# ykojima4020/mae_clip

Measured on NVIDIA B200. Metric: contrastive loss fwd+bwd samples/s, higher is better.
Workload: dtype fp32 (fp16 hi+lo split operands, 3 tcgen05 passes, fp32 accumulate)

## Files before the change

mae_clip_b200/csrc/clip_loss_tc.cu:

```cuda
#include <stdlib.h>
#include <string.h>

#include "clip_loss.cuh"
#include "tc_ptx.cuh"

#include <type_traits>

namespace mc {
namespace tc {

using namespace ptx;


constexpr int kTileN = 128;
constexpr int kRowsCta = 64;
constexpr int kChunkBytes = 64 * 128;
constexpr int kThreads = 384;
constexpr int kEpiThreads = 256;
constexpr int kMaxSplit = 16;
constexpr int kIssuers = 1;

enum Phase { kStats = 0, kRowLoss = 1, kBwd = 2, kStatsZ = 3, kBwdW = 4, kBwdP = 5 };

constexpr int kOffA = 0;
// ... 1206 lines not shown
                                                           float* __restrict__ dT, float* __restrict__ dI,
                                                           const int* __restrict__ gate = nullptr, int gate_want = 0) {
  if (gate != nullptr && *gate != gate_want) return;
  const float scale = (grad_loss ? *grad_loss : 1.f) * inv_2B / *wscale;
  const size_t n4 = (size_t)b * D / 4;
  const size_t plane = (size_t)bpad * D;
  for (size_t i = (size_t)blockIdx.x * blockDim.x + threadIdx.x; i < n4; i += (size_t)gridDim.x * blockDim.x) {
    float4 at = make_float4(0.f, 0.f, 0.f, 0.f), ai = at;
    for (int s = 0; s < nsplit; ++s) {
      const float4 a = reinterpret_cast<const float4*>(part + (size_t)s * 2 * plane)[i];
      const float4 c = reinterpret_cast<const float4*>(part + ((size_t)s * 2 + 1) * plane)[i];
      at.x += a.x; at.y += a.y; at.z += a.z; at.w += a.w;
      ai.x += c.x; ai.y += c.y; ai.z += c.z; ai.w += c.w;
    }
    reinterpret_cast<float4*>(dT)[i] = make_float4(at.x * scale, at.y * scale, at.z * scale, at.w * scale);
    reinterpret_cast<float4*>(dI)[i] = make_float4(ai.x * scale, ai.y * scale, ai.z * scale, ai.w * scale);
  }
}

constexpr int kCgThreads = 256;
constexpr int kCgStageA = 2 * 8192;
constexpr int kCgStages = 6;
constexpr int kCgMaxSplit = 8;
struct ColGradParams {
  int Bp, D;
  int w_rows;
  int row_offset;
  int j_first;
  int n_jblocks;
  int j_end;
  int ksplit, steps_per_split, steps;
  float* part;
  const int* gate;
};
__device__ __forceinline__ uint64_t smem_desc_mn_sw128(uint32_t saddr, uint32_t lbo_bytes) {
  uint64_t d = 0;
  d |= static_cast<uint64_t>((saddr & 0x3FFFFu) >> 4);
  d |= static_cast<uint64_t>(lbo_bytes >> 4) << 16;
  d |= static_cast<uint64_t>(1024 >> 4) << 32;
  d |= static_cast<uint64_t>(1) << 46;
  d |= static_cast<uint64_t>(2) << 61;
  return d;
}
__global__ void __launch_bounds__(kCgThreads, 1)
colgrad_kernel(const __grid_constant__ CUtensorMap map_w, const __grid_constant__ CUtensorMap map_t,
               const ColGradParams p) {
  if (p.gate != nullptr && *p.gate != 1) return;
  extern __shared__ uint8_t smem_raw[];
  const uint32_t raw = smem_u32(smem_raw);
  const uint32_t base = (raw + 1023u) & ~1023u;
  uint8_t* const sbase = smem_raw + (base - raw);
  const int D = p.D;
  const uint32_t b_bytes = (uint32_t)(D / 2) * 128u;
  const uint32_t stage_bytes = kCgStageA + b_bytes;
  const uint32_t bar0 = base + kCgStages * stage_bytes;
  auto bar = [&](int i) -> uint32_t { return bar0 + 8u * i; };
  enum { kFull = 0, kEmpty = kCgStages, kAccFull = 2 * kCgStages, kAccEmpty = 2 * kCgStages + 2, kBars = 2 * kCgStages + 4 };
  uint32_t* const tmem_slot = reinterpret_cast<uint32_t*>(sbase + kCgStages * stage_bytes + 8 * kBars);

  const int warp = __shfl_sync(0xffffffffu, (int)(threadIdx.x >> 5), 0), lane = threadIdx.x & 31;
  const uint32_t rank = cluster_ctarank();
  const bool leader = rank == 0;
  const int pair_id = blockIdx.x >> 1, npairs = gridDim.x >> 1;
  const int njobs = p.n_jblocks * p.ksplit;

  if (threadIdx.x == 0) {
    for (int s = 0; s < kCgStages; ++s) { mbar_init(bar(kFull + s), 1); mbar_init(bar(kEmpty + s), 1); }
    for (int i = 0; i < 2; ++i) { mbar_init(bar(kAccFull + i), 1); mbar_init(bar(kAccEmpty + i), 2 * 128); }
    fence_mbar_init();
    prefetch_tmap(&map_w);
    prefetch_tmap(&map_t);
  }
  if (warp == 1) {
    tmem_alloc_pair(smem_u32(tmem_slot), 512);
    tmem_relinquish_pair();
  }
  tc_fence_before();
  cluster_sync_all();
  tc_fence_after();
  const uint32_t tmem_base = *tmem_slot;

  if (warp == 0) {
    if (elect_one()) {
      uint32_t it = 0;
      for (int job = pair_id; job < njobs; job += npairs) {
        const int jb = job / p.ksplit, ks = job % p.ksplit;
        const int j0 = p.j_first + jb * 256 + (int)rank * 128;
        const int s0 = ks * p.steps_per_split, s1 = min(s0 + p.steps_per_split, p.steps);
        for (int st = s0; st < s1; ++st, ++it) {
          const uint32_t slot = it % kCgStages, par = (it / kCgStages) & 1;
          mbar_wait(bar(kEmpty + slot), par ^ 1);
          const uint32_t fb = bar(kFull + slot), sa = base + slot * stage_bytes;
          if (leader) mbar_arrive_expect_tx(fb, 2u * stage_bytes);
          const int i0 = st * 64;
          tma_load_2d_pair(sa, &map_w, fb, j0, i0);
          tma_load_2d_pair(sa + 8192, &map_w, fb, j0 + 64, i0);
          tma_load_2d_pair(sa + kCgStageA, &map_t, fb, p.row_offset + i0, D + (int)rank * (D / 2));
        }
      }
    }
  } else if (warp == 1) {
    if (leader && elect_one()) {
      const uint32_t idesc = idesc_f16(256, D) | (1u << 15);
      uint32_t it = 0, jj = 0;
      for (int job = pair_id; job < njobs; job += npairs) {
        const int ks = job % p.ksplit;
        const int s0 = ks * p.steps_per_split, s1 = min(s0 + p.steps_per_split, p.steps);
        if (s0 >= s1) continue;
        const uint32_t buf = jj & 1, use = jj >> 1;
        ++jj;
        mbar_wait(bar(kAccEmpty + buf), (use & 1) ^ 1);
        tc_fence_after();
        const uint32_t tacc = tmem_base + buf * (uint32_t)D;
        for (int st = s0; st < s1; ++st, ++it) {
          const uint32_t slot = it % kCgStages, par = (it / kCgStages) & 1;
          mbar_wait(bar(kFull + slot), par);
          tc_fence_after();
          const uint32_t sa = base + slot * stage_bytes;
          const uint64_t bd = smem_desc_sw128(sa + kCgStageA);
#pragma unroll
          for (int k4 = 0; k4 < 4; ++k4)
            mma_f16_pair(tacc, smem_desc_mn_sw128(sa + k4 * 2048, 8192), desc_advance_k(bd, k4), idesc,
                         (st > s0 || k4 > 0) ? 1u : 0u);
          mma_commit_pair(bar(kEmpty + slot), 3);
        }
        mma_commit_pair(bar(kAccFull + buf), 3);
      }
    }
  } else if (warp >= 4) {
// ... 82 lines not shown
                                                                int rows, int D, float inv_2B,
                                                                const float* __restrict__ grad_loss,
                                                                const float* __restrict__ wscale,
                                                                const float* __restrict__ dIz, float* __restrict__ dI,
                                                                const int* __restrict__ gate) {
  if (gate != nullptr && *gate != 1) return;
  const float scale = (grad_loss ? *grad_loss : 1.f) * inv_2B / *wscale;
  const size_t n4 = (size_t)rows * D / 4;
  for (size_t i = (size_t)blockIdx.x * blockDim.x + threadIdx.x; i < n4; i += (size_t)gridDim.x * blockDim.x) {
    float4 a = dIz ? reinterpret_cast<const float4*>(dIz)[i] : make_float4(0.f, 0.f, 0.f, 0.f);
    for (int s = 0; s < ksplit; ++s) {
      const float4 c = reinterpret_cast<const float4*>(part + (size_t)s * plane)[i];
      a.x += c.x; a.y += c.y; a.z += c.z; a.w += c.w;
    }
    reinterpret_cast<float4*>(dI)[i] = make_float4(a.x * scale, a.y * scale, a.z * scale, a.w * scale);
  }
}

constexpr int kRgThreads = 384;
constexpr int kRgRowsCta = 128;
constexpr int kRgSlotBytes = 32768;
constexpr int kRgSlots = 3;
constexpr int kRgOffA = 0;
constexpr int kRgOffRing = 65536;
constexpr int kRgOffW = kRgOffRing + kRgSlots * kRgSlotBytes;
constexpr int kRgOffXT = kRgOffW + 2 * 16384;
constexpr int kRgOffConst = kRgOffXT + 2 * 16384;
constexpr int kRgOffBar = kRgOffConst + 2048;
constexpr int kRgSmemBytes = kRgOffBar + 256 + 512;
enum RgBar {
  kRgFull0 = 0, kRgEmpty0 = 3, kRgAFull = 6, kRgJobDone = 7, kRgTmemFull0 = 8, kRgTmemEmpty0 = 10, kRgWFull0 = 12,
  kRgXTFull0 = 14, kRgGradDone0 = 16, kRgAccFull = 18, kRgAccEmpty = 19, kRgCstFull0 = 20, kRgCstEmpty0 = 22, kRgNumBars = 24
};
struct RowGradParams {
  int b, B, Bp, D, row_offset;
  int n_row_blocks, n_tiles, nsplit, tiles_per_split, bpad;
  float inv_tau;
  const float* scale;
  const float *r, *c, *q;
  const float* wscale;
  float* part;
  __half* wout;
  const int* gate;
};
template <int PASSES>
__global__ void __launch_bounds__(kRgThreads, 1)
rowgrad_kernel(const __grid_constant__ CUtensorMap map_a_hi, const __grid_constant__ CUtensorMap map_a_lo,
               const __grid_constant__ CUtensorMap map_b_hi, const __grid_constant__ CUtensorMap map_b_lo,
               const __grid_constant__ CUtensorMap map_t, const RowGradParams p) {
  if (p.gate != nullptr && *p.gate != 1) return;
  extern __shared__ __align__(1024) uint8_t smem_raw[];
  const uint32_t raw = smem_u32(smem_raw);
  const uint32_t base = (raw + 1023u) & ~1023u;
  if (base - raw > 512u) __trap();
  uint8_t* const sbase = smem_raw + (base - raw);
  const uint32_t bar0 = base + kRgOffBar;
  auto bar = [&](int i) -> uint32_t { return bar0 + 8u * i; };
  uint32_t* const tmem_slot = reinterpret_cast<uint32_t*>(sbase + kRgOffBar + 8 * kRgNumBars);

  const int warp = __shfl_sync(0xffffffffu, (int)(threadIdx.x >> 5), 0), lane = threadIdx.x & 31;
  const uint32_t rank = cluster_ctarank();
  const bool leader = rank == 0;
  const int pair_id = blockIdx.x >> 1, npairs = gridDim.x >> 1;
  const int D = p.D, nkc = D >> 6;
  const int njobs = p.n_row_blocks * p.nsplit;
  const uint32_t xt_bytes = (uint32_t)(D / 2) * 128u;

  if (threadIdx.x == 0) {
    for (int s = 0; s < kRgSlots; ++s) { mbar_init(bar(kRgFull0 + s), 1); mbar_init(bar(kRgEmpty0 + s), 1); }
    mbar_init(bar(kRgAFull), 1);
    mbar_init(bar(kRgJobDone), 1);
    for (int i = 0; i < 2; ++i) {
      mbar_init(bar(kRgTmemFull0 + i), 1);
      mbar_init(bar(kRgTmemEmpty0 + i), 2 * 256);
      mbar_init(bar(kRgWFull0 + i), 2 * 128);
      mbar_init(bar(kRgXTFull0 + i), 1);
      mbar_init(bar(kRgGradDone0 + i), 1);
      mbar_init(bar(kRgCstFull0 + i), 32);
      mbar_init(bar(kRgCstEmpty0 + i), 256);
    }
    mbar_init(bar(kRgAccFull), 1);
    mbar_init(bar(kRgAccEmpty), 2 * 256);
    fence_mbar_init();
    prefetch_tmap(&map_a_hi); prefetch_tmap(&map_a_lo); prefetch_tmap(&map_b_hi); prefetch_tmap(&map_b_lo);
    prefetch_tmap(&map_t);
  }
  if (warp == 1) {
    tmem_alloc_pair(smem_u32(tmem_slot), 512);
    tmem_relinquish_pair();
  }
  tc_fence_before();
  cluster_sync_all();
  tc_fence_after();
  const uint32_t tmem_base = *tmem_slot;
  constexpr uint32_t kAcc = 256;

  if (warp == 0) {
    if (elect_one()) {
      uint32_t it = 0, jj = 0;
      for (int job = pair_id; job < njobs; job += npairs, ++jj) {
        const int rb = job / p.nsplit, sp = job % p.nsplit;
        const int row_a = p.row_offset + rb * 256 + (int)rank * kRgRowsCta;
        const int t0 = sp * p.tiles_per_split, t1 = min(t0 + p.tiles_per_split, p.n_tiles);
        mbar_wait(bar(kRgJobDone), (jj & 1) ^ 1);
        if (leader) mbar_arrive_expect_tx(bar(kRgAFull), 2u * (uint32_t)nkc * 16384u);
        for (int c = 0; c < nkc; ++c) tma_load_2d_pair(base + kRgOffA + c * 16384, &map_a_hi, bar(kRgAFull), D + c * 64, row_a);
        for (int t = t0; t < t1; ++t) {
          const int j0 = t * kTileN + 64 * (int)rank;
          for (int c = 0; c < nkc; ++c, ++it) {
            const uint32_t slot = it % kRgSlots, par = (it / kRgSlots) & 1;
            mbar_wait(bar(kRgEmpty0 + slot), par ^ 1);
            const uint32_t fb = bar(kRgFull0 + slot), sb = base + kRgOffRing + slot * kRgSlotBytes;
            if (leader) mbar_arrive_expect_tx(fb, PASSES == 3 ? 2u * kRgSlotBytes : 2u * 8192u);
            if (PASSES == 3) tma_load_2d_pair(sb, &map_a_lo, fb, D + c * 64, row_a);
            tma_load_2d_pair(sb + 16384, &map_b_hi, fb, c * 64, j0);
            if (PASSES == 3) tma_load_2d_pair(sb + 24576, &map_b_lo, fb, c * 64, j0);
          }
        }
      }
    }
  } else if (warp == 2) {
    if (elect_one()) {
      uint32_t tt = 0;
      for (int job = pair_id; job < njobs; job += npairs) {
        const int sp = job % p.nsplit;
        const int t0 = sp * p.tiles_per_split, t1 = min(t0 + p.tiles_per_split, p.n_tiles);
        for (int t = t0; t < t1; ++t, ++tt) {
          for (int h = 0; h < 2; ++h) {
            mbar_wait(bar(kRgGradDone0 + h), (tt & 1) ^ 1);
            const uint32_t fb = bar(kRgXTFull0 + h);
            if (leader) mbar_arrive_expect_tx(fb, 2u * xt_bytes);
            tma_load_2d_pair(base + kRgOffXT + h * 16384, &map_t, fb, t * kTileN + 64 * h, (int)rank * (D / 2));
          }
        }
      }
    }
  } else if (warp == 3) {
    float* const consts = reinterpret_cast<float*>(sbase + kRgOffConst);
    const float kL2e = 1.4426950408889634f;
    const bool fast = p.wscale[1] != 0.f;
    const float m_rc = p.wscale[2];
    uint32_t tt = 0;
    for (int job = pair_id; job < njobs; job += npairs) {
      const int sp = job % p.nsplit;
      const int t0 = sp * p.tiles_per_split, t1 = min(t0 + p.tiles_per_split, p.n_tiles);
      for (int t = t0; t < t1; ++t, ++tt) {
        float vc[4], vq[4];
#pragma unroll
        for (int u = 0; u < 4; ++u) {
          const int jcol = t * kTileN + lane + 32 * u;
          const bool ok = jcol < p.B;
          vc[u] = ok ? p.c[jcol] : 0.f;
          vq[u] = ok ? p.q[jcol] : 0.f;
        }
        mbar_wait(bar(kRgCstEmpty0 + (tt & 1)), ((tt >> 1) & 1) ^ 1);
        float* dst = consts + (tt & 1) * 256;
#pragma unroll
        for (int u = 0; u < 4; ++u) {
          const int col = lane + 32 * u;
          const bool ok = t * kTileN + col < p.B;
          const float c2 = vc[u] * kL2e;
          if (fast) {
            dst[col] = ok ? ex2f(m_rc - c2) * vq[u] : 0.f;
          } else {
            dst[col] = -c2;
            dst[128 + col] = vq[u];
          }
        }
        mbar_arrive_local(bar(kRgCstFull0 + (tt & 1)));
      }
    }
  } else if (warp == 1) {
    if (leader && elect_one()) {
      constexpr uint32_t idesc_s = idesc_f16(256, kTileN);
      const uint32_t idesc_g = idesc_f16(256, D);
      const uint32_t tDT = tmem_base + kAcc;
      uint32_t it = 0, tt = 0, gt = 0, jj = 0;
      auto grad_tile = [&](bool first_of_job) {
        for (int h = 0; h < 2; ++h) {
          mbar_wait(bar(kRgWFull0 + h), gt & 1);
          mbar_wait(bar(kRgXTFull0 + h), gt & 1);
          tc_fence_after();
          const uint64_t wd = smem_desc_sw128(base + kRgOffW + h * 16384), xd = smem_desc_sw128(base + kRgOffXT + h * 16384);
#pragma unroll
          for (int ks = 0; ks < 4; ++ks)
            mma_f16_pair(tDT, desc_advance_k(wd, ks), desc_advance_k(xd, ks), idesc_g, (first_of_job && h == 0 && ks == 0) ? 0u : 1u);
          mma_commit_pair(bar(kRgGradDone0 + h), 3);
        }
        ++gt;
      };
      for (int job = pair_id; job < njobs; job += npairs, ++jj) {
        const int sp = job % p.nsplit;
        const int t0 = sp * p.tiles_per_split, t1 = min(t0 + p.tiles_per_split, p.n_tiles);
        mbar_wait(bar(kRgAFull), jj & 1);
        tc_fence_after();
        for (int t = t0; t < t1; ++t, ++tt) {
          const uint32_t buf = tt & 1, use = tt >> 1;
          mbar_wait(bar(kRgTmemEmpty0 + buf), (use & 1) ^ 1);
          tc_fence_after();
          const uint32_t tS = tmem_base + buf * 128;
          for (int c = 0; c < nkc; ++c, ++it) {
            const uint32_t slot = it % kRgSlots, par = (it / kRgSlots) & 1;
            mbar_wait(bar(kRgFull0 + slot), par);
            tc_fence_after();
            const uint32_t sb = base + kRgOffRing + slot * kRgSlotBytes;
            const uint64_t aT = smem_desc_sw128(base + kRgOffA + c * 16384), aTl = smem_desc_sw128(sb);
            const uint64_t bI = smem_desc_sw128(sb + 16384), bIl = smem_desc_sw128(sb + 24576);
#pragma unroll
            for (int ks = 0; ks < 4; ++ks) {
              const uint64_t kT = desc_advance_k(aT, ks), kb = desc_advance_k(bI, ks);
              mma_f16_pair(tS, kT, kb, idesc_s, (c > 0 || ks > 0) ? 1u : 0u);
              if (PASSES == 3) {
                mma_f16_pair(tS, kT, desc_advance_k(bIl, ks), idesc_s, 1u);
                mma_f16_pair(tS, desc_advance_k(aTl, ks), kb, idesc_s, 1u);
              }
            }
            mma_commit_pair(bar(kRgEmpty0 + slot), 3);
          }
          mma_commit_pair(bar(kRgTmemFull0 + buf), 3);
          if (t == t0) {
            mbar_wait(bar(kRgAccEmpty), (jj & 1) ^ 1);
            tc_fence_after();
          } else {
            grad_tile(t - 1 == t0);
          }
        }
        grad_tile(t1 - 1 == t0);
        mma_commit_pair(bar(kRgAccFull), 3);
        mma_commit_pair(bar(kRgJobDone), 3);
      }
    }
    __syncwarp();
  } else if (warp >= 4) {
    const int q4 = warp & 3, h = (warp - 4) >> 2;
    const int m = q4 * 32 + lane;
    const uint32_t lane_field = (uint32_t)(q4 * 32) << 16;
    const float* const consts = reinterpret_cast<const float*>(sbase + kRgOffConst);
    const float kL2e = 1.4426950408889634f;
    const float inv_s = p.scale[1], inv_s2 = p.scale[2];
    const float cS2 = inv_s2 * p.inv_tau * kL2e;
    const float wS = inv_s * p.inv_tau * p.wscale[0];
    const bool fast = p.wscale[1] != 0.f;
    const float m_rc = p.wscale[2];
    uint32_t tt = 0, jj = 0;
    for (int job = pair_id; job < njobs; job += npairs, ++jj) {
      const int rb = job / p.nsplit, sp = job % p.nsplit;
      const int t0 = sp * p.tiles_per_split, t1 = min(t0 + p.tiles_per_split, p.n_tiles);
      const int lrow = rb * 256 + (int)rank * kRgRowsCta + m;
      const int gi = p.row_offset + lrow;
      const bool row_ok = lrow < p.b;
      const float r2_i = row_ok ? p.r[gi] * kL2e : 0.f;
      const float fC_i = ex2f(r2_i - m_rc);
      const float wrow = row_ok ? wS : 0.f;
      for (int t = t0; t < t1; ++t, ++tt) {
        const uint32_t buf = tt & 1, use = tt >> 1;
        mbar_wait(bar(kRgCstFull0 + (tt & 1)), (tt >> 1) & 1);
        const float* cst = consts + (tt & 1) * 256 + 64 * h;
        mbar_wait(bar(kRgTmemFull0 + buf), use & 1);
        tc_fence_after();
        const uint32_t tS = tmem_base + buf * 128 + lane_field + 64 * h;
        const bool ragged = (t + 1) * kTileN > p.B;
        uint32_t wp[32];
#pragma unroll
        for (int half = 0; half < 2; ++half) {
          float v[32];
          tmem_ld32(tS + 32 * half, v);
          tmem_ld_wait();
          if (half == 1) {
            tc_fence_before();
            mbar_arrive_cluster(bar(kRgTmemEmpty0 + buf), 0);
          }
#pragma unroll
          for (int e = 0; e < 32; e += 4) {
            const float4 f0 = *reinterpret_cast<const float4*>(cst + 32 * half + e);
            const float4 f1 = fast ? make_float4(0.f, 0.f, 0.f, 0.f) : *reinterpret_cast<const float4*>(cst + 128 + 32 * half + e);
            const float k0[4] = {f0.x, f0.y, f0.z, f0.w}, k1[4] = {f1.x, f1.y, f1.z, f1.w};
            float w[4];
#pragma unroll
            for (int u = 0; u < 4; ++u) {
              const float a = v[e + u];
              const float e1 = ex2f(fmaf(a, cS2, -r2_i));
              float dS;
              if (fast) dS = e1 * fmaf(fC_i, k0[u], 1.f);
              else dS = fmaf(ex2f(fmaf(a, cS2, k0[u])), k1[u], e1);
              w[u] = dS * wrow;
            }
            __half2 x = __floats2half2_rn(w[0], w[1]), y = __floats2half2_rn(w[2], w[3]);
            wp[16 * half + (e >> 1)] = *reinterpret_cast<uint32_t*>(&x);
            wp[16 * half + (e >> 1) + 1] = *reinterpret_cast<uint32_t*>(&y);
          }
        }
        mbar_wait(bar(kRgGradDone0 + h), (tt & 1) ^ 1);
        uint8_t* wsm = sbase + kRgOffW + h * 16384 + m * 128;
#pragma unroll
        for (int k = 0; k < 8; ++k)
          *reinterpret_cast<uint4*>(wsm + ((k ^ (m & 7)) * 16)) = make_uint4(wp[4 * k], wp[4 * k + 1], wp[4 * k + 2], wp[4 * k + 3]);
        if (ragged) zero_padding_cols(wsm, m, max(p.B - t * kTileN - 64 * h, 0), 64);
        fence_proxy_async_smem();
        mbar_arrive_cluster(bar(kRgWFull0 + h), 0);
        uint4* wg = reinterpret_cast<uint4*>(p.wout + (size_t)lrow * p.Bp + (size_t)t * kTileN + 64 * h);
#pragma unroll
        for (int k = 0; k < 8; ++k) wg[k] = make_uint4(wp[4 * k], wp[4 * k + 1], wp[4 * k + 2], wp[4 * k + 3]);
        mbar_arrive_local(bar(kRgCstEmpty0 + (tt & 1)));
      }
      mbar_wait(bar(kRgAccFull), jj & 1);
      tc_fence_after();
      float* out = p.part + ((size_t)sp * p.bpad + lrow) * D + h * (D / 2);
      for (int c0 = 0; c0 < D / 2; c0 += 32) {
        float v[32];
        tmem_ld32(tmem_base + lane_field + kAcc + h * (D / 2) + c0, v);
        tmem_ld_wait();
#pragma unroll
        for (int e = 0; e < 32; e += 4) *reinterpret_cast<float4*>(out + c0 + e) = make_float4(v[e], v[e + 1], v[e + 2], v[e + 3]);
      }
      tc_fence_before();
      mbar_arrive_cluster(bar(kRgAccEmpty), 0);
    }
  }
  tc_fence_before();
  cluster_sync_all();
  if (warp == 1) tmem_dealloc_pair(tmem_base, 512);
}

enum RsKind { kRsS = 0, kRsZ = 1 };
constexpr int kRsThreads = 384;
constexpr int kRsNBuf = 4;
constexpr int kRsOffScratch = 212992;
constexpr int kRsOffBar = kRsOffScratch + 2048;
constexpr int kRsSmemBytes = kRsOffBar + 256 + 512;
enum RsBar { kRsFull0 = 0, kRsEmpty0 = 5, kRsAFull = 10, kRsJobDone = 11, kRsTmemFull0 = 12, kRsTmemEmpty0 = 16, kRsNumBars = 20 };
struct RowSweepParams {
  int b, B, Bp, D, row_offset;
  int n_row_blocks, n_tiles, nsplit, tiles_per_split, bpad;
  int chunk_k, chunk_blocks, chunk_m;
  int tri;
  float inv_tau, half_tau;
  const float* scale;
  float2* part;
  float* colpart;
  uint8_t* flags_out;
  const float *norm_i, *norm_t;
  const float* tile_min_zjj2;
  int pk;
  const float* rho;
  const float* tile_max_rho;
  const float* tile_max_n;
  const int* gate;
  int gate_want;
};
__device__ __forceinline__ int rs_njobs(const RowSweepParams& p) {
// ... 1193 lines not shown
  for (int k = 1; k <= kCgMaxSplit && k <= c.steps; ++k) {
    const int per = (c.steps + k - 1) / k;
    const long jobs = (long)c.n_jblocks * k;
    const double cost = (double)((jobs + npairs - 1) / npairs) * (per + 16.0) + 4.0 * k;
    if (cost < best_cost - 1e-9) { best_cost = cost; best = k; }
  }
  c.ksplit = best;
  c.steps_per_split = (c.steps + best - 1) / best;
  return c;
}
const float* bwd_rows_wscale(void* ws, int b, int B, int D) { return wscale_slot(ws, b, B, D); }
size_t stored_weights_bytes(int b, int B) { return round_up(round_up((size_t)b, 256) * round_up((size_t)B, 128) * sizeof(__half), 256); }
size_t bwd_cols_workspace_bytes(int , int n_cols, int D) {
  return round_up((size_t)kCgMaxSplit * ((size_t)(n_cols + 255) / 256 * 256) * D * sizeof(float), 256) + 256;
}
StoredLayout stored_layout(int B, int D, int mode) {
  StoredLayout l;
  l.off_w = round_up(core_workspace_bytes(B, B, D, mode), 1024);
  l.off_diz = l.off_w + stored_weights_bytes(B, B);
  l.off_cols = l.off_diz + round_up(round_up((size_t)B, 128) * D * sizeof(float), 256);
  l.cols_bytes = bwd_cols_workspace_bytes(B, B, D);
  l.total = l.off_cols + l.cols_bytes;
  return l;
}
size_t workspace_bytes(int b, int B, int D, int mode) {
  if (b == B && stored_form_enabled(b, B, D)) return stored_layout(B, D, mode).total;
  return core_workspace_bytes(b, B, D, mode);
}
bool stored_form_enabled(int b, int B, int D) {
  static const bool off = getenv("MAE_CLIP_BWD_FORM") != nullptr && strcmp(getenv("MAE_CLIP_BWD_FORM"), "ownrows") == 0;
  return !off && supported(D) && (double)b * (double)B >= 4096.0 * 4096.0 && stored_weights_bytes(b, B) <= ((size_t)16 << 30);
}

static int launch_rowgrad(const ClipProblem& p, int mode, const ClipStatsAll& s, float* part, const float* wscale,
                          __half* wout, cudaStream_t st) {
  MC_REQUIRE(p.row_offset % 128 == 0, MC_ERR_UNSUPPORTED, "rowgrad: row_offset %% 128 != 0 (%d)", p.row_offset);
  PlanesLayout l = planes_layout(p.B, p.D);
  const char* base = static_cast<const char*>(p.planes_all);
  const void* Xh = base + l.off_hi;
  const void* Xl = base + l.off_lo;
  CUtensorMap ma_hi, ma_lo, mb_hi, mb_lo, mt;
  int rc;
  if ((rc = make_map(&ma_hi, Xh, l.Bp, 2 * p.D, 128))) return rc;
  if ((rc = make_map(&ma_lo, Xl, l.Bp, 2 * p.D, 128))) return rc;
  if ((rc = make_map(&mb_hi, Xh, l.Bp, 2 * p.D, 64))) return rc;
  if ((rc = make_map(&mb_lo, Xl, l.Bp, 2 * p.D, 64))) return rc;
  if ((rc = make_map(&mt, base + l.off_hiT, 2 * p.D, l.Bp, p.D / 2))) return rc;
  Split sp = choose_split_rows256(p.b, p.B);
  RowGradParams rp;
  rp.b = p.b; rp.B = p.B; rp.Bp = l.Bp; rp.D = p.D; rp.row_offset = p.row_offset;
  rp.n_row_blocks = sp.n_row_blocks; rp.n_tiles = sp.n_tiles; rp.nsplit = sp.nsplit;
  rp.tiles_per_split = sp.tiles_per_split; rp.bpad = sp.bpad;
  rp.inv_tau = 1.f / p.tau;
  rp.scale = reinterpret_cast<const float*>(base + l.off_hdr) + 1;
  rp.r = s.r; rp.c = s.c; rp.q = s.q;
  rp.wscale = wscale;
  rp.part = part;
  rp.wout = wout;
  rp.gate = p.gate;
  const bool three = mode == MC_GEMM_TC_F16X3;
  static std::atomic<unsigned long long> attr_done3{0}, attr_done1{0};
  if (three) MC_CUDA(ensure_dynamic_smem(rowgrad_kernel<3>, kRgSmemBytes, attr_done3));
  else MC_CUDA(ensure_dynamic_smem(rowgrad_kernel<1>, kRgSmemBytes, attr_done1));
  const long njobs = (long)sp.n_row_blocks * sp.nsplit;
  int npairs = num_sms() / 2;
  if (njobs < npairs) npairs = (int)njobs;
  cudaLaunchConfig_t cfg = {};
  cfg.gridDim = dim3(2 * npairs);
  cfg.blockDim = dim3(kRgThreads);
  cfg.dynamicSmemBytes = kRgSmemBytes;
  cfg.stream = st;
  cudaLaunchAttribute attr[1];
  attr[0].id = cudaLaunchAttributeClusterDimension;
  attr[0].val.clusterDim.x = 2;
  attr[0].val.clusterDim.y = 1;
  attr[0].val.clusterDim.z = 1;
  cfg.attrs = attr;
  cfg.numAttrs = 1;
  if (three) MC_CUDA(cudaLaunchKernelEx(&cfg, rowgrad_kernel<3>, ma_hi, ma_lo, mb_hi, mb_lo, mt, rp));
  else MC_CUDA(cudaLaunchKernelEx(&cfg, rowgrad_kernel<1>, ma_hi, ma_lo, mb_hi, mb_lo, mt, rp));
  count_launch();
  return MC_OK;
}

__global__ void __launch_bounds__(1024) bwd_gate_kernel(const uint8_t* __restrict__ flags, size_t n, float thresh, int* __restrict__ gate) {
  __shared__ unsigned int sm[32];
  unsigned int cnt = 0;
  size_t i0 = 0;
  if ((reinterpret_cast<uintptr_t>(flags) & 15) == 0) {
    const size_t n16 = n >> 4;
    for (size_t i = threadIdx.x; i < n16; i += blockDim.x) {
      const uint4 v = reinterpret_cast<const uint4*>(flags)[i];
      cnt += (__popc(__vcmpne4(v.x, 0u)) + __popc(__vcmpne4(v.y, 0u)) + __popc(__vcmpne4(v.z, 0u)) + __popc(__vcmpne4(v.w, 0u))) >> 3;
    }
    i0 = n16 << 4;
  }
  for (size_t i = i0 + threadIdx.x; i < n; i += blockDim.x) cnt += flags[i] != 0;
  for (int o = 16; o > 0; o >>= 1) cnt += __shfl_xor_sync(0xffffffffu, cnt, o);
  if ((threadIdx.x & 31) == 0) sm[threadIdx.x >> 5] = cnt;
  __syncthreads();
  if (threadIdx.x < 32) {
    cnt = sm[threadIdx.x];
    for (int o = 16; o > 0; o >>= 1) cnt += __shfl_xor_sync(0xffffffffu, cnt, o);
    if (threadIdx.x == 0) *gate = ((float)cnt <= thresh * (float)n) ? 1 : 0;
  }
}
int bwd_gate(const uint8_t* flags, size_t n_flags, int* gate_out, cudaStream_t st) {
  static const float thresh = getenv("MAE_CLIP_BWD_GATE") ? (float)atof(getenv("MAE_CLIP_BWD_GATE")) : 0.15f;
  bwd_gate_kernel<<<1, 1024, 0, st>>>(flags, n_flags, thresh, gate_out);
  MC_LAUNCH_CHECK();
  return MC_OK;
}

// ... 42 lines not shown
  return MC_OK;
}

int bwd_cols(const ClipProblem& p, int mode, const ClipStatsAll& s, const float* grad_loss, const void* W, int w_rows,
             int w_row_offset, int j0, int j1, const float* dIz, float* dI_out, void* ws, size_t ws_bytes, cudaStream_t st,
             const float* wscale_ready) {
  (void)mode;
  MC_REQUIRE(supported(p.D), MC_ERR_UNSUPPORTED, "clip_bwd_cols: D %d", p.D);
  MC_REQUIRE(j0 % 128 == 0 && j0 >= 0 && j1 > j0 && j1 <= p.B && w_rows > 0 && w_row_offset % 64 == 0, MC_ERR_BAD_ARG,
             "clip_bwd_cols: bad ranges (j %d..%d, rows %d at %d)", j0, j1, w_rows, w_row_offset);
  MC_REQUIRE(ws_bytes >= bwd_cols_workspace_bytes(w_rows, j1 - j0, p.D), MC_ERR_WORKSPACE, "clip_bwd_cols: workspace too small");
  MC_REQUIRE(aligned(W, 256) && aligned(dI_out, 16) && (!dIz || aligned(dIz, 16)), MC_ERR_ALIGN, "clip_bwd_cols: alignment");
  PlanesLayout l = planes_layout(p.B, p.D);
  const char* base = static_cast<const char*>(p.planes_all);
  const int w_rows_pad = (int)round_up((size_t)w_rows, 128);
  CUtensorMap mw, mt;
  int rc;
  if ((rc = make_map(&mw, W, w_rows_pad, l.Bp, 64))) return rc;
  if ((rc = make_map(&mt, base + l.off_hiT, 2 * p.D, l.Bp, p.D / 2))) return rc;
  ColSplit cs = choose_col_split(w_rows_pad, j1 - j0);
  const size_t part_bytes = round_up((size_t)kCgMaxSplit * ((size_t)cs.n_jblocks * 256) * p.D * sizeof(float), 256);
  const float* wsc = wscale_ready;
  if (wsc == nullptr) {
    float* w2 = reinterpret_cast<float*>(static_cast<char*>(ws) + part_bytes);
    if ((rc = launch_wscale(p, s, w2, st))) return rc;
    wsc = w2;
  }
  ColGradParams cp;
  cp.Bp = l.Bp; cp.D = p.D; cp.w_rows = w_rows_pad; cp.row_offset = w_row_offset;
  cp.j_first = j0; cp.n_jblocks = cs.n_jblocks; cp.j_end = j1;
  cp.ksplit = cs.ksplit; cp.steps_per_split = cs.steps_per_split; cp.steps = cs.steps;
  cp.part = static_cast<float*>(ws);
  cp.gate = p.gate;
  const int smem = kCgStages * (kCgStageA + (p.D / 2) * 128) + 8 * 32 + 16 + 1024;
  const int smem_max = kCgStages * (kCgStageA + 128 * 128) + 8 * 32 + 16 + 1024;
  static std::atomic<unsigned long long> attr_done{0};
  MC_CUDA(ensure_dynamic_smem(colgrad_kernel, smem_max, attr_done));
  const long njobs = (long)cs.n_jblocks * cs.ksplit;
  int npairs = num_sms() / 2;
  if (njobs < npairs) npairs = (int)njobs;
  cudaLaunchConfig_t cfg = {};
  cfg.gridDim = dim3(2 * npairs);
  cfg.blockDim = dim3(kCgThreads);
  cfg.dynamicSmemBytes = smem;
  cfg.stream = st;
  cudaLaunchAttribute attr[1];
  attr[0].id = cudaLaunchAttributeClusterDimension;
  attr[0].val.clusterDim.x = 2;
  attr[0].val.clusterDim.y = 1;
  attr[0].val.clusterDim.z = 1;
  cfg.attrs = attr;
  cfg.numAttrs = 1;
  MC_CUDA(cudaLaunchKernelEx(&cfg, colgrad_kernel, mw, mt, cp));
  count_launch();
  const int rows = j1 - j0;
  size_t n4 = (size_t)rows * p.D / 4;
  int blocks = (int)((n4 + 255) / 256);
  int cap = num_sms() * 8;
  if (blocks > cap) blocks = cap;
  bwd_cols_finalize_kernel<<<blocks, 256, 0, st>>>(static_cast<const float*>(ws), cs.ksplit, (size_t)cs.n_jblocks * 256 * p.D,
                                                   rows, p.D, 0.5f / (float)p.B, grad_loss, wsc, dIz, dI_out, p.gate);
  MC_LAUNCH_CHECK();
  return MC_OK;
}

}
// ... 2 lines not shown
```

mae_clip_b200/csrc/tc_ptx.cuh:

```cuda
#pragma once

#include <cuda.h>
#include <cuda_fp16.h>
#include <cuda_runtime.h>
#include <stdint.h>
#include <stdio.h>

namespace mc {
namespace ptx {

__device__ __forceinline__ uint32_t smem_u32(const void* p) {
  return static_cast<uint32_t>(__cvta_generic_to_shared(p));
}
__device__ __forceinline__ uint32_t cluster_ctarank() {
  uint32_t r;
  asm volatile("mov.u32 %0, %%cluster_ctarank;" : "=r"(r));
  return r;
}
__device__ __forceinline__ void cluster_sync_all() {
  asm volatile("barrier.cluster.arrive.release.aligned;\n\tbarrier.cluster.wait.acquire.aligned;" ::: "memory");
}
__device__ __forceinline__ bool elect_one() {
  uint32_t pred;
  asm volatile(
// ... 37 lines not shown
}
__device__ __forceinline__ void mbar_wait(uint32_t bar, uint32_t parity) {
  if (mbar_try_wait(bar, parity)) return;
  const long long t0 = clock64();
  while (!mbar_try_wait(bar, parity)) {
    if (clock64() - t0 > 4000000000LL) mbar_timeout(bar, parity);
  }
}

__device__ __forceinline__ void fence_proxy_async_smem() {
  asm volatile("fence.proxy.async.shared::cta;" ::: "memory");
}
__device__ __forceinline__ void tc_fence_before() {
  asm volatile("tcgen05.fence::before_thread_sync;" ::: "memory");
}
__device__ __forceinline__ void tc_fence_after() {
  asm volatile("tcgen05.fence::after_thread_sync;" ::: "memory");
}
__device__ __forceinline__ void named_bar_sync(uint32_t id, uint32_t threads) {
  asm volatile("bar.sync %0, %1;" ::"r"(id), "r"(threads) : "memory");
}

__device__ __forceinline__ void prefetch_tmap(const CUtensorMap* m) {
  asm volatile("prefetch.tensormap [%0];" ::"l"(reinterpret_cast<uint64_t>(m)) : "memory");
}
constexpr uint32_t kPeerBitMask = 0xFEFFFFFFu;
__device__ __forceinline__ void tma_load_2d_pair(uint32_t smem_dst, const CUtensorMap* map, uint32_t bar,
                                                 int c0, int c1) {
  asm volatile(
      "cp.async.bulk.tensor.2d.cta_group::2.shared::cluster.global.mbarrier::complete_tx::bytes"
      " [%0], [%1, {%3, %4}], [%2];" ::"r"(smem_dst),
      "l"(reinterpret_cast<uint64_t>(map)), "r"(bar & kPeerBitMask), "r"(c0), "r"(c1)
      : "memory");
}

__device__ __forceinline__ void tmem_alloc_pair(uint32_t dst_smem, uint32_t cols) {
  asm volatile("tcgen05.alloc.cta_group::2.sync.aligned.shared::cta.b32 [%0], %1;" ::"r"(dst_smem), "r"(cols)
               : "memory");
}
__device__ __forceinline__ void tmem_relinquish_pair() {
  asm volatile("tcgen05.relinquish_alloc_permit.cta_group::2.sync.aligned;" ::: "memory");
}
__device__ __forceinline__ void tmem_dealloc_pair(uint32_t taddr, uint32_t cols) {
  asm volatile("tcgen05.dealloc.cta_group::2.sync.aligned.b32 %0, %1;" ::"r"(taddr), "r"(cols) : "memory");
}

__device__ __forceinline__ void mma_f16_pair(uint32_t tmem_d, uint64_t adesc, uint64_t bdesc, uint32_t idesc,
                                             uint32_t accumulate) {
  asm volatile(
      "{\n\t.reg .pred p;\n\tsetp.ne.b32 p, %4, 0;\n\t"
      "tcgen05.mma.cta_group::2.kind::f16 [%0], %1, %2, %3, p;\n\t}" ::"r"(tmem_d),
      "l"(adesc), "l"(bdesc), "r"(idesc), "r"(accumulate)
      : "memory");
}
__device__ __forceinline__ void mma_commit_pair(uint32_t bar, uint16_t mask) {
  asm volatile(
      "tcgen05.commit.cta_group::2.mbarrier::arrive::one.shared::cluster.multicast::cluster.b64 [%0], %1;" ::"r"(bar),
      "h"(mask)
      : "memory");
}

__device__ __forceinline__ void tmem_ld32(uint32_t taddr, float* v) {
  uint32_t* r = reinterpret_cast<uint32_t*>(v);
  asm volatile(
      "tcgen05.ld.sync.aligned.32x32b.x32.b32 "
      "{%0, %1, %2, %3, %4, %5, %6, %7, %8, %9, %10, %11, %12, %13, %14, %15, "
// ... 59 lines not shown
```

Before: 8.549 million.

## Store rowgrad weight tiles via TMA with evict-first hint, evict-first colgrad reads

The rowgrad epilogue now writes the fp16 weight tile from the already-staged swizzled shared-memory buffer with a TMA bulk store carrying an L2 evict_first policy, replacing per-thread global uint4 stores. Named barriers and bulk read-waits guard reuse of that buffer. The colgrad kernel loads the weights back with the same evict_first hint, so the streamed weight matrix is meant not to push other data out of L2. A plain-store fallback is kept behind an environment variable, and profiling wait hooks were added alongside.

```diff
diff --git a/mae_clip_b200/csrc/clip_loss_tc.cu b/mae_clip_b200/csrc/clip_loss_tc.cu
--- a/mae_clip_b200/csrc/clip_loss_tc.cu
+++ b/mae_clip_b200/csrc/clip_loss_tc.cu
@@ -1262,6 +1262,7 @@
   int ksplit, steps_per_split, steps;
   float* part;
   const int* gate;
+  int w_evict_first;
 };
 __device__ __forceinline__ uint64_t smem_desc_mn_sw128(uint32_t saddr, uint32_t lbo_bytes) {
   uint64_t d = 0;
@@ -1312,6 +1313,7 @@
 
   if (warp == 0) {
     if (elect_one()) {
+      const uint64_t w_policy = l2_policy_evict_first();
       uint32_t it = 0;
       for (int job = pair_id; job < njobs; job += npairs) {
         const int jb = job / p.ksplit, ks = job % p.ksplit;
@@ -1323,8 +1325,13 @@
           const uint32_t fb = bar(kFull + slot), sa = base + slot * stage_bytes;
           if (leader) mbar_arrive_expect_tx(fb, 2u * stage_bytes);
           const int i0 = st * 64;
-          tma_load_2d_pair(sa, &map_w, fb, j0, i0);
-          tma_load_2d_pair(sa + 8192, &map_w, fb, j0 + 64, i0);
+          if (p.w_evict_first) {
+            tma_load_2d_pair_hint(sa, &map_w, fb, j0, i0, w_policy);
+            tma_load_2d_pair_hint(sa + 8192, &map_w, fb, j0 + 64, i0, w_policy);
+          } else {
+            tma_load_2d_pair(sa, &map_w, fb, j0, i0);
+            tma_load_2d_pair(sa + 8192, &map_w, fb, j0 + 64, i0);
+          }
           tma_load_2d_pair(sa + kCgStageA, &map_t, fb, p.row_offset + i0, D + (int)rank * (D / 2));
         }
       }
@@ -1473,6 +1480,8 @@
   kRgFull0 = 0, kRgEmpty0 = 3, kRgAFull = 6, kRgJobDone = 7, kRgTmemFull0 = 8, kRgTmemEmpty0 = 10, kRgWFull0 = 12,
   kRgXTFull0 = 14, kRgGradDone0 = 16, kRgAccFull = 18, kRgAccEmpty = 19, kRgCstFull0 = 20, kRgCstEmpty0 = 22, kRgNumBars = 24
 };
+enum RgProf { kRgProfIssuer = 32, kRgProfProducer = 40, kRgProfEpi = 48 };
+enum RgWStore { kRgWStoreTma = 0, kRgWStorePlain = 1 };
 struct RowGradParams {
   int b, B, Bp, D, row_offset;
   int n_row_blocks, n_tiles, nsplit, tiles_per_split, bpad;
@@ -1483,12 +1492,13 @@
   float* part;
   __half* wout;
   const int* gate;
+  int wstore;
 };
 template <int PASSES>
 __global__ void __launch_bounds__(kRgThreads, 1)
 rowgrad_kernel(const __grid_constant__ CUtensorMap map_a_hi, const __grid_constant__ CUtensorMap map_a_lo,
                const __grid_constant__ CUtensorMap map_b_hi, const __grid_constant__ CUtensorMap map_b_lo,
-               const __grid_constant__ CUtensorMap map_t, const RowGradParams p) {
+               const __grid_constant__ CUtensorMap map_t, const __grid_constant__ CUtensorMap map_w, const RowGradParams p) {
   if (p.gate != nullptr && *p.gate != 1) return;
   extern __shared__ __align__(1024) uint8_t smem_raw[];
   const uint32_t raw = smem_u32(smem_raw);
@@ -1525,6 +1535,7 @@
     fence_mbar_init();
     prefetch_tmap(&map_a_hi); prefetch_tmap(&map_a_lo); prefetch_tmap(&map_b_hi); prefetch_tmap(&map_b_lo);
     prefetch_tmap(&map_t);
+    if (p.wstore == kRgWStoreTma) prefetch_tmap(&map_w);
   }
   if (warp == 1) {
     tmem_alloc_pair(smem_u32(tmem_slot), 512);
@@ -1538,19 +1549,20 @@
 
   if (warp == 0) {
     if (elect_one()) {
+      [[maybe_unused]] const long long prof_t0 = MC_PROF_NOW();
       uint32_t it = 0, jj = 0;
       for (int job = pair_id; job < njobs; job += npairs, ++jj) {
         const int rb = job / p.nsplit, sp = job % p.nsplit;
         const int row_a = p.row_offset + rb * 256 + (int)rank * kRgRowsCta;
         const int t0 = sp * p.tiles_per_split, t1 = min(t0 + p.tiles_per_split, p.n_tiles);
-        mbar_wait(bar(kRgJobDone), (jj & 1) ^ 1);
+        mbar_wait_t(bar(kRgJobDone), (jj & 1) ^ 1, kRgProfProducer + 2, leader);
         if (leader) mbar_arrive_expect_tx(bar(kRgAFull), 2u * (uint32_t)nkc * 16384u);
         for (int c = 0; c < nkc; ++c) tma_load_2d_pair(base + kRgOffA + c * 16384, &map_a_hi, bar(kRgAFull), D + c * 64, row_a);
         for (int t = t0; t < t1; ++t) {
           const int j0 = t * kTileN + 64 * (int)rank;
           for (int c = 0; c < nkc; ++c, ++it) {
             const uint32_t slot = it % kRgSlots, par = (it / kRgSlots) & 1;
-            mbar_wait(bar(kRgEmpty0 + slot), par ^ 1);
+            mbar_wait_t(bar(kRgEmpty0 + slot), par ^ 1, kRgProfProducer + 1, leader);
             const uint32_t fb = bar(kRgFull0 + slot), sb = base + kRgOffRing + slot * kRgSlotBytes;
             if (leader) mbar_arrive_expect_tx(fb, PASSES == 3 ? 2u * kRgSlotBytes : 2u * 8192u);
             if (PASSES == 3) tma_load_2d_pair(sb, &map_a_lo, fb, D + c * 64, row_a);
@@ -1559,6 +1571,7 @@
           }
         }
       }
+      MC_PROF_TOTAL(kRgProfProducer, prof_t0, leader);
     }
   } else if (warp == 2) {
     if (elect_one()) {
@@ -1613,14 +1626,15 @@
     }
   } else if (warp == 1) {
     if (leader && elect_one()) {
+      [[maybe_unused]] const long long prof_t0 = MC_PROF_NOW();
       constexpr uint32_t idesc_s = idesc_f16(256, kTileN);
       const uint32_t idesc_g = idesc_f16(256, D);
       const uint32_t tDT = tmem_base + kAcc;
       uint32_t it = 0, tt = 0, gt = 0, jj = 0;
       auto grad_tile = [&](bool first_of_job) {
         for (int h = 0; h < 2; ++h) {
-          mbar_wait(bar(kRgWFull0 + h), gt & 1);
-          mbar_wait(bar(kRgXTFull0 + h), gt & 1);
+          mbar_wait_t(bar(kRgWFull0 + h), gt & 1, kRgProfIssuer + 3, true);
+          mbar_wait_t(bar(kRgXTFull0 + h), gt & 1, kRgProfIssuer + 4, true);
           tc_fence_after();
           const uint64_t wd = smem_desc_sw128(base + kRgOffW + h * 16384), xd = smem_desc_sw128(base + kRgOffXT + h * 16384);
 #pragma unroll
@@ -1633,16 +1647,16 @@
       for (int job = pair_id; job < njobs; job += npairs, ++jj) {
         const int sp = job % p.nsplit;
         const int t0 = sp * p.tiles_per_split, t1 = min(t0 + p.tiles_per_split, p.n_tiles);
-        mbar_wait(bar(kRgAFull), jj & 1);
+        mbar_wait_t(bar(kRgAFull), jj & 1, kRgProfIssuer + 6, true);
         tc_fence_after();
         for (int t = t0; t < t1; ++t, ++tt) {
           const uint32_t buf = tt & 1, use = tt >> 1;
-          mbar_wait(bar(kRgTmemEmpty0 + buf), (use & 1) ^ 1);
+          mbar_wait_t(bar(kRgTmemEmpty0 + buf), (use & 1) ^ 1, kRgProfIssuer + 1, true);
           tc_fence_after();
           const uint32_t tS = tmem_base + buf * 128;
           for (int c = 0; c < nkc; ++c, ++it) {
             const uint32_t slot = it % kRgSlots, par = (it / kRgSlots) & 1;
-            mbar_wait(bar(kRgFull0 + slot), par);
+            mbar_wait_t(bar(kRgFull0 + slot), par, kRgProfIssuer + 2, true);
             tc_fence_after();
             const uint32_t sb = base + kRgOffRing + slot * kRgSlotBytes;
             const uint64_t aT = smem_desc_sw128(base + kRgOffA + c * 16384), aTl = smem_desc_sw128(sb);
@@ -1660,7 +1674,7 @@
           }
           mma_commit_pair(bar(kRgTmemFull0 + buf), 3);
           if (t == t0) {
-            mbar_wait(bar(kRgAccEmpty), (jj & 1) ^ 1);
+            mbar_wait_t(bar(kRgAccEmpty), (jj & 1) ^ 1, kRgProfIssuer + 5, true);
             tc_fence_after();
           } else {
             grad_tile(t - 1 == t0);
@@ -1670,6 +1684,7 @@
         mma_commit_pair(bar(kRgAccFull), 3);
         mma_commit_pair(bar(kRgJobDone), 3);
       }
+      MC_PROF_TOTAL(kRgProfIssuer, prof_t0, true);
     }
     __syncwarp();
   } else if (warp >= 4) {
@@ -1683,6 +1698,11 @@
     const float wS = inv_s * p.inv_tau * p.wscale[0];
     const bool fast = p.wscale[1] != 0.f;
     const float m_rc = p.wscale[2];
+    const int wstore = p.wstore;
+    const uint64_t w_policy = l2_policy_evict_first();
+    [[maybe_unused]] const int prof_base = kRgProfEpi + 8 * h;
+    [[maybe_unused]] const bool prof_rec = leader && m == 0;
+    [[maybe_unused]] const long long prof_t0 = MC_PROF_NOW();
     uint32_t tt = 0, jj = 0;
     for (int job = pair_id; job < njobs; job += npairs, ++jj) {
       const int rb = job / p.nsplit, sp = job % p.nsplit;
@@ -1693,11 +1713,12 @@
       const float r2_i = row_ok ? p.r[gi] * kL2e : 0.f;
       const float fC_i = ex2f(r2_i - m_rc);
       const float wrow = row_ok ? wS : 0.f;
+      const bool w_row = lrow < ((p.b + 127) & ~127);
       for (int t = t0; t < t1; ++t, ++tt) {
         const uint32_t buf = tt & 1, use = tt >> 1;
-        mbar_wait(bar(kRgCstFull0 + (tt & 1)), (tt >> 1) & 1);
+        mbar_wait_t(bar(kRgCstFull0 + (tt & 1)), (tt >> 1) & 1, prof_base + 3, prof_rec);
         const float* cst = consts + (tt & 1) * 256 + 64 * h;
-        mbar_wait(bar(kRgTmemFull0 + buf), use & 1);
+        mbar_wait_t(bar(kRgTmemFull0 + buf), use & 1, prof_base + 1, prof_rec);
         tc_fence_after();
         const uint32_t tS = tmem_base + buf * 128 + lane_field + 64 * h;
         const bool ragged = (t + 1) * kTileN > p.B;
@@ -1731,7 +1752,11 @@
             wp[16 * half + (e >> 1) + 1] = *reinterpret_cast<uint32_t*>(&y);
           }
         }
-        mbar_wait(bar(kRgGradDone0 + h), (tt & 1) ^ 1);
+        mbar_wait_t(bar(kRgGradDone0 + h), (tt & 1) ^ 1, prof_base + 2, prof_rec);
+        if (wstore == kRgWStoreTma) {
+          if (m == 0) bulk_wait_group_read0();
+          named_bar_sync(1 + h, 128);
+        }
         uint8_t* wsm = sbase + kRgOffW + h * 16384 + m * 128;
 #pragma unroll
         for (int k = 0; k < 8; ++k)
@@ -1739,12 +1764,22 @@
         if (ragged) zero_padding_cols(wsm, m, max(p.B - t * kTileN - 64 * h, 0), 64);
         fence_proxy_async_smem();
         mbar_arrive_cluster(bar(kRgWFull0 + h), 0);
-        uint4* wg = reinterpret_cast<uint4*>(p.wout + (size_t)lrow * p.Bp + (size_t)t * kTileN + 64 * h);
-#pragma unroll
-        for (int k = 0; k < 8; ++k) wg[k] = make_uint4(wp[4 * k], wp[4 * k + 1], wp[4 * k + 2], wp[4 * k + 3]);
+#ifndef MC_ABLATE_WSTORE
+        if (wstore == kRgWStoreTma) {
+          named_bar_sync(1 + h, 128);
+          if (m == 0) {
+            tma_store_2d_hint(&map_w, base + kRgOffW + h * 16384, t * kTileN + 64 * h, rb * 256 + (int)rank * kRgRowsCta, w_policy);
+            bulk_commit_group();
+          }
+        } else if (w_row) {
+          uint4* wg = reinterpret_cast<uint4*>(p.wout + (size_t)lrow * p.Bp + (size_t)t * kTileN + 64 * h);
+#pragma unroll
+          for (int k = 0; k < 8; ++k) wg[k] = make_uint4(wp[4 * k], wp[4 * k + 1], wp[4 * k + 2], wp[4 * k + 3]);
+        }
+#endif
         mbar_arrive_local(bar(kRgCstEmpty0 + (tt & 1)));
       }
-      mbar_wait(bar(kRgAccFull), jj & 1);
+      mbar_wait_t(bar(kRgAccFull), jj & 1, prof_base + 4, prof_rec);
       tc_fence_after();
       float* out = p.part + ((size_t)sp * p.bpad + lrow) * D + h * (D / 2);
       for (int c0 = 0; c0 < D / 2; c0 += 32) {
@@ -1757,6 +1792,8 @@
       tc_fence_before();
       mbar_arrive_cluster(bar(kRgAccEmpty), 0);
     }
+    if (wstore == kRgWStoreTma && m == 0) bulk_wait_group0();
+    MC_PROF_TOTAL(prof_base, prof_t0, prof_rec);
   }
   tc_fence_before();
   cluster_sync_all();
@@ -3016,6 +3053,11 @@
   return !off && supported(D) && (double)b * (double)B >= 4096.0 * 4096.0 && stored_weights_bytes(b, B) <= ((size_t)16 << 30);
 }
 
+static int rg_wstore() {
+  const char* e = getenv("MAE_CLIP_RG_WSTORE");
+  return e != nullptr && strcmp(e, "plain") == 0 ? kRgWStorePlain : kRgWStoreTma;
+}
+
 static int launch_rowgrad(const ClipProblem& p, int mode, const ClipStatsAll& s, float* part, const float* wscale,
                           __half* wout, cudaStream_t st) {
   MC_REQUIRE(p.row_offset % 128 == 0, MC_ERR_UNSUPPORTED, "rowgrad: row_offset %% 128 != 0 (%d)", p.row_offset);
@@ -3023,7 +3065,7 @@
   const char* base = static_cast<const char*>(p.planes_all);
   const void* Xh = base + l.off_hi;
   const void* Xl = base + l.off_lo;
-  CUtensorMap ma_hi, ma_lo, mb_hi, mb_lo, mt;
+  CUtensorMap ma_hi, ma_lo, mb_hi, mb_lo, mt, mw;
   int rc;
   if ((rc = make_map(&ma_hi, Xh, l.Bp, 2 * p.D, 128))) return rc;
   if ((rc = make_map(&ma_lo, Xl, l.Bp, 2 * p.D, 128))) return rc;
@@ -3042,6 +3084,8 @@
   rp.part = part;
   rp.wout = wout;
   rp.gate = p.gate;
+  rp.wstore = rg_wstore();
+  if ((rc = make_map(&mw, wout, round_up((size_t)p.b, 128), l.Bp, kRgRowsCta))) return rc;
   const bool three = mode == MC_GEMM_TC_F16X3;
   static std::atomic<unsigned long long> attr_done3{0}, attr_done1{0};
   if (three) MC_CUDA(ensure_dynamic_smem(rowgrad_kernel<3>, kRgSmemBytes, attr_done3));
@@ -3061,8 +3105,8 @@
   attr[0].val.clusterDim.z = 1;
   cfg.attrs = attr;
   cfg.numAttrs = 1;
-  if (three) MC_CUDA(cudaLaunchKernelEx(&cfg, rowgrad_kernel<3>, ma_hi, ma_lo, mb_hi, mb_lo, mt, rp));
-  else MC_CUDA(cudaLaunchKernelEx(&cfg, rowgrad_kernel<1>, ma_hi, ma_lo, mb_hi, mb_lo, mt, rp));
+  if (three) MC_CUDA(cudaLaunchKernelEx(&cfg, rowgrad_kernel<3>, ma_hi, ma_lo, mb_hi, mb_lo, mt, mw, rp));
+  else MC_CUDA(cudaLaunchKernelEx(&cfg, rowgrad_kernel<1>, ma_hi, ma_lo, mb_hi, mb_lo, mt, mw, rp));
   count_launch();
   return MC_OK;
 }
@@ -3171,6 +3215,7 @@
   cp.ksplit = cs.ksplit; cp.steps_per_split = cs.steps_per_split; cp.steps = cs.steps;
   cp.part = static_cast<float*>(ws);
   cp.gate = p.gate;
+  cp.w_evict_first = rg_wstore() == kRgWStoreTma;
   const int smem = kCgStages * (kCgStageA + (p.D / 2) * 128) + 8 * 32 + 16 + 1024;
   const int smem_max = kCgStages * (kCgStageA + 128 * 128) + 8 * 32 + 16 + 1024;
   static std::atomic<unsigned long long> attr_done{0};
diff --git a/mae_clip_b200/csrc/tc_ptx.cuh b/mae_clip_b200/csrc/tc_ptx.cuh
--- a/mae_clip_b200/csrc/tc_ptx.cuh
+++ b/mae_clip_b200/csrc/tc_ptx.cuh
@@ -93,6 +93,31 @@
       " [%0], [%1, {%3, %4}], [%2];" ::"r"(smem_dst),
       "l"(reinterpret_cast<uint64_t>(map)), "r"(bar & kPeerBitMask), "r"(c0), "r"(c1)
       : "memory");
+}
+__device__ __forceinline__ void tma_load_2d_pair_hint(uint32_t smem_dst, const CUtensorMap* map, uint32_t bar,
+                                                      int c0, int c1, uint64_t policy) {
+  asm volatile(
+      "cp.async.bulk.tensor.2d.cta_group::2.shared::cluster.global.mbarrier::complete_tx::bytes.L2::cache_hint"
+      " [%0], [%1, {%3, %4}], [%2], %5;" ::"r"(smem_dst),
+      "l"(reinterpret_cast<uint64_t>(map)), "r"(bar & kPeerBitMask), "r"(c0), "r"(c1), "l"(policy)
+      : "memory");
+}
+__device__ __forceinline__ void tma_store_2d_hint(const CUtensorMap* map, uint32_t smem_src, int c0, int c1,
+                                                  uint64_t policy) {
+  asm volatile(
+      "cp.async.bulk.tensor.2d.global.shared::cta.bulk_group.L2::cache_hint [%0, {%2, %3}], [%1], %4;" ::"l"(
+          reinterpret_cast<uint64_t>(map)),
+      "r"(smem_src), "r"(c0), "r"(c1), "l"(policy)
+      : "memory");
+}
+__device__ __forceinline__ void bulk_commit_group() { asm volatile("cp.async.bulk.commit_group;" ::: "memory"); }
+__device__ __forceinline__ void bulk_wait_group_read0() { asm volatile("cp.async.bulk.wait_group.read 0;" ::: "memory"); }
+__device__ __forceinline__ void bulk_wait_group0() { asm volatile("cp.async.bulk.wait_group 0;" ::: "memory"); }
+
+__device__ __forceinline__ uint64_t l2_policy_evict_first() {
+  uint64_t pol;
+  asm volatile("createpolicy.fractional.L2::evict_first.b64 %0, 1.0;" : "=l"(pol));
+  return pol;
 }
 
 __device__ __forceinline__ void tmem_alloc_pair(uint32_t dst_smem, uint32_t cols) {
```

Result: faster. 9.242 million (median of 6 runs) (+8.1%).
